# MayDomine/Burst-Attention

Hardware: NVIDIA H100
Metric: attention fwd+bwd TFLOPS/s (bs=1, H=32, d=128, bf16; seq in config, default 262144 on N > 1 GPUs, 65536 on one), aggregate over GPUs (higher is better)
Workload: dtype bf16

## Files before the change

burst-attention_b200/csrc/bwd_sm90.cu:

```cuda
#include <math.h>
#include <stdlib.h>

#include <mutex>
#include <vector>

#include "host_common.h"
#include "sm90_ptx.cuh"

namespace ba {

constexpr int kBwdThreads = 384;
constexpr int kBwdN = 128;
constexpr int kBwdM = 64;

struct BwdParams {
  const float* lse;
  int64_t lse_sb, lse_sh;
  const float* delta;
  int64_t dl_sb, dl_sh;
  float* dk_acc;
  int64_t dk_sb, dk_ss, dk_sh;
  float* dv_acc;
  int64_t dv_sb, dv_ss, dv_sh;
  int B, Sq, Sk, H;
  int G;
  float scale, scale_log2;
  int causal, causal_off;
  const float* bias;
  int64_t bias_sb, bias_sh;
  int* sem;
  int* ticket;
};

__device__ __forceinline__ int ld_acquire_gpu(const int* p) {
  int v;
  asm volatile("ld.acquire.gpu.global.s32 %0, [%1];" : "=r"(v) : "l"(p) : "memory");
  return v;
}
__device__ __forceinline__ void st_release_gpu(int* p, int v) {
  asm volatile("st.release.gpu.global.s32 [%0], %1;" ::"l"(p), "r"(v) : "memory");
}

struct __align__(8) BwdBarriers {
  uint64_t kv_full;
  uint64_t q_full[2], q_empty[2];
  int key_block;
};

template <int kD>
struct BwdLayout {
  static_assert(kD == 64 || kD == 128, "head dim 64 or 128");
  static constexpr int kBoxes = kD / 64;
  static constexpr int kBoxKV = kBwdN * 128;
  static constexpr int kBoxQ = kBwdM * 128;
  static constexpr int kOffK = 0;
  static constexpr int kOffV = kOffK + kBoxes * kBoxKV;
  static constexpr int kOffQ = kOffV + kBoxes * kBoxKV;
  static constexpr int kOffDO = kOffQ + 2 * kBoxes * kBoxQ;
  static constexpr int kOffDS = kOffDO + 2 * kBoxes * kBoxQ;
  static constexpr int kOffDQ = kOffDS + 2 * kBwdN * 128;
  static constexpr int kOffStat = kOffDQ + kBoxes * kBwdM * 64 * 4;
  static constexpr int kOffBar = kOffStat + 2 * 2 * kBwdM * 4;
  static constexpr int kSmemBytes = kOffBar + 64;
  static_assert(kSmemBytes <= 232448, "backward kernel exceeds 227 KiB of shared memory");
};

template <bool kBF16, int kD>
__global__ void __launch_bounds__(kBwdThreads, 1)
bwd_chunk_kernel(const __grid_constant__ CUtensorMap tmQ, const __grid_constant__ CUtensorMap tmK,
                 const __grid_constant__ CUtensorMap tmV, const __grid_constant__ CUtensorMap tmDO,
                 const __grid_constant__ CUtensorMap tmDQ, const BwdParams p) {
  extern __shared__ __align__(1024) uint8_t smem_raw[];
  uint8_t* smem = smem_raw;
  if ((smem_u32(smem) & 1023u) != 0) __trap();
  using L = BwdLayout<kD>;
  constexpr int kBoxes = L::kBoxes, kBoxKV = L::kBoxKV, kBoxQ = L::kBoxQ, kAcc = kD / 2;
  constexpr int kQStageB = kBoxes * kBoxQ;
  float* sStat = reinterpret_cast<float*>(smem + L::kOffStat);
  BwdBarriers* bars = reinterpret_cast<BwdBarriers*>(smem + L::kOffBar);

  const int warp = __shfl_sync(0xffffffffu, threadIdx.x >> 5, 0);
  const int lane = threadIdx.x & 31;
  const int hk = blockIdx.y, b = blockIdx.z;
  const int h0 = hk * p.G;
  int kb = blockIdx.x;
// ... 21 lines not shown
      mbar_init(&bars->q_empty[s], 8);
    }
    fence_mbar_init();
  }
  __syncthreads();

  if (warp < 4) {
    reg_alloc_dec<24>();
    if (warp != 0) return;
    if (lane == 0) {
      mbar_arrive_expect_tx(&bars->kv_full, 2 * kBoxes * kBoxKV);
      for (int half = 0; half < kBoxes; ++half) {
        tma_load_4d(smem + L::kOffK + half * kBoxKV, &tmK, &bars->kv_full, half * 64, hk, k0, b);
        tma_load_4d(smem + L::kOffV + half * kBoxKV, &tmV, &bars->kv_full, half * 64, hk, k0, b);
      }
    }
    int it = 0, h = h0;
    for (int step = 0; step < n_steps; ++step) {
      const int q0 = (i_begin + it) * kBwdM;
      const int st = step & 1;
      mbar_wait(&bars->q_empty[st], ((step >> 1) & 1) ^ 1);
      float* stat = sStat + st * 2 * kBwdM;
#pragma unroll
      for (int j = 0; j < 2; ++j) {
        const int row = q0 + lane + 32 * j;
        float l = INFINITY, dl = 0.f;
        if (row < p.Sq) {
          l = __ldg(p.lse + (int64_t)b * p.lse_sb + (int64_t)h * p.lse_sh + row);
          dl = __ldg(p.delta + (int64_t)b * p.dl_sb + (int64_t)h * p.dl_sh + row);
          if (l == -INFINITY) l = INFINITY;
        }
        stat[lane + 32 * j] = l * kLog2e;
        stat[kBwdM + lane + 32 * j] = dl;
      }
      __syncwarp();
      if (lane == 0) {
        mbar_arrive_expect_tx(&bars->q_full[st], 2 * kQStageB);
        for (int half = 0; half < kBoxes; ++half) {
          tma_load_4d(smem + L::kOffQ + st * kQStageB + half * kBoxQ, &tmQ, &bars->q_full[st], half * 64, h, q0, b);
          tma_load_4d(smem + L::kOffDO + st * kQStageB + half * kBoxQ, &tmDO, &bars->q_full[st], half * 64, h, q0, b);
        }
      }
      __syncwarp();
      if (++it == n_it) it = 0, ++h;
    }
    return;
  }

  reg_alloc_inc<240>();
  const int wg = (threadIdx.x >> 7) - 1;
  const int tid = threadIdx.x & 127;
  const int w = warp & 3, g = lane >> 2, t = lane & 3;
  const int kr_lo = wg * 64 + 16 * w + g;
  const int keys[2] = {k0 + kr_lo, k0 + kr_lo + 8};
  const float scale_log2 = p.scale_log2;
  float bias2[2];
  const bool reducer = kD == 128 || wg == 0;
  const int n_red = kD == 128 ? 2 : 1;

  float dk[kAcc], dv[kAcc];
#pragma unroll
  for (int i = 0; i < kAcc; ++i) dk[i] = dv[i] = 0.f;

  const uint32_t sK = smem_u32(smem + L::kOffK), sV = smem_u32(smem + L::kOffV);
  const uint32_t kw = wg * 64 * 128;
  float* sDQ = reinterpret_cast<float*>(smem + L::kOffDQ) + wg * kBwdM * 64;
  mbar_wait(&bars->kv_full, 0);
  int it = 0, h = h0;
  for (int step = 0; step < n_steps; ++step) {
    const int q0 = (i_begin + it) * kBwdM;
    const int st = step & 1;
    const uint32_t sQ = smem_u32(smem + L::kOffQ + st * kQStageB), sDO = smem_u32(smem + L::kOffDO + st * kQStageB);
    const float* stat = sStat + st * 2 * kBwdM;
    if (it == 0) {
#pragma unroll
      for (int r = 0; r < 2; ++r)
        bias2[r] = (p.bias && keys[r] < p.Sk)
                       ? __ldg(p.bias + (int64_t)b * p.bias_sb + (int64_t)h * p.bias_sh + keys[r]) * kLog2e
                       : 0.f;
    }
    mbar_wait(&bars->q_full[st], (step >> 1) & 1);

    float s[32], dp[32];
    wgmma_fence();
#pragma unroll
    for (int kk = 0; kk < kD / 16; ++kk) {
      const uint32_t okv = (kk >> 2) * kBoxKV + kw + (kk & 3) * 32, oq = (kk >> 2) * kBoxQ + (kk & 3) * 32;
      wgmma_ss_n64<kBF16, 0, 0>(s, make_desc(sK + okv, 16, 1024), make_desc(sQ + oq, 16, 1024), kk > 0 ? 1u : 0u);
    }
    wgmma_commit();
#pragma unroll
    for (int kk = 0; kk < kD / 16; ++kk) {
      const uint32_t okv = (kk >> 2) * kBoxKV + kw + (kk & 3) * 32, oq = (kk >> 2) * kBoxQ + (kk & 3) * 32;
      wgmma_ss_n64<kBF16, 0, 0>(dp, make_desc(sV + okv, 16, 1024), make_desc(sDO + oq, 16, 1024), kk > 0 ? 1u : 0u);
    }
    wgmma_commit();
    wgmma_wait<1>();
    fence_regs<32>(s);

    const bool need_mask = p.causal && (q0 + p.causal_off < k0 + kBwdN - 1);
    uint32_t pp[16], ds[16];
#pragma unroll
    for (int c = 0; c < 8; ++c) {
      const float2 l2 = *reinterpret_cast<const float2*>(stat + 8 * c + 2 * t);
#pragma unroll
      for (int r = 0; r < 2; ++r) {
        const int e = 4 * c + 2 * r;
        float p0 = ex2(fmaf(s[e], scale_log2, bias2[r] - l2.x));
        float p1 = ex2(fmaf(s[e + 1], scale_log2, bias2[r] - l2.y));
        if (keys[r] >= p.Sk) p0 = p1 = 0.f;
        if (need_mask) {
          const int q = q0 + 8 * c + 2 * t;
          if (q < keys[r] - p.causal_off) p0 = 0.f;
          if (q + 1 < keys[r] - p.causal_off) p1 = 0.f;
        }
        s[e] = p0, s[e + 1] = p1;
        pp[2 * c + r] = pack2<kBF16>(p0, p1);
      }
    }

    wgmma_wait<0>();
    fence_regs<32>(dp);
    fence_regs<16>(pp);
    fence_regs<kAcc>(dv);
    wgmma_fence();
#pragma unroll
    for (int kk = 0; kk < kBwdM / 16; ++kk) {
      const uint64_t d_do = make_desc(sDO + kk * 16 * 128, kBoxQ, 1024);
      if constexpr (kD == 128) wgmma_rs_n128<kBF16, 1>(dv, pp + 4 * kk, d_do, 1u);
      else wgmma_rs_n64<kBF16, 1>(dv, pp + 4 * kk, d_do, 1u);
    }
    wgmma_commit();

#pragma unroll
    for (int c = 0; c < 8; ++c) {
      const float2 dl = *reinterpret_cast<const float2*>(stat + kBwdM + 8 * c + 2 * t);
#pragma unroll
      for (int r = 0; r < 2; ++r) {
        const int e = 4 * c + 2 * r;
        ds[2 * c + r] = pack2<kBF16>(s[e] * (dp[e] - dl.x), s[e + 1] * (dp[e + 1] - dl.y));
      }
    }

    uint8_t* sDS = smem + L::kOffDS + st * kBwdN * 128;
#pragma unroll
    for (int c = 0; c < 8; ++c)
#pragma unroll
      for (int r = 0; r < 2; ++r) {
        const int kr = kr_lo + 8 * r;
        *reinterpret_cast<uint32_t*>(sDS + kr * 128 + ((c ^ (kr & 7)) << 4) + 4 * t) = ds[2 * c + r];
      }
    fence_proxy_async_smem();
    named_bar_sync(1, 256);

    float dq[32];
    fence_regs<16>(ds);
    fence_regs<kAcc>(dk);
    auto issue_dk = [&]() {
#pragma unroll
      for (int kk = 0; kk < kBwdM / 16; ++kk) {
        const uint64_t d_q = make_desc(sQ + kk * 16 * 128, kBoxQ, 1024);
        if constexpr (kD == 128) wgmma_rs_n128<kBF16, 1>(dk, ds + 4 * kk, d_q, 1u);
        else wgmma_rs_n64<kBF16, 1>(dk, ds + 4 * kk, d_q, 1u);
      }
      wgmma_commit();
    };
    if (reducer) {
      const uint32_t a0 = smem_u32(sDS), b0 = sK + wg * kBoxKV;
      wgmma_fence();
#pragma unroll
      for (int kk = 0; kk < kBwdN / 16; ++kk)
        wgmma_ss_n64<kBF16, 1, 1>(dq, make_desc(a0 + kk * 16 * 128, 8192, 1024),
                                  make_desc(b0 + kk * 16 * 128, kBoxKV, 1024), kk > 0 ? 1u : 0u);
      wgmma_commit();
      issue_dk();
      wgmma_wait<1>();
    } else {
      wgmma_fence();
      issue_dk();
      wgmma_wait<1>();
    }
    fence_regs<kAcc>(dv);
    fence_regs<16>(pp);

    if (reducer) {
      fence_regs<32>(dq);
      const uint32_t bar_id = 2 + wg;
      if (tid == 0) tma_store_wait_read<0>();
      named_bar_sync(bar_id, 128);
#pragma unroll
      for (int c = 0; c < 8; ++c)
#pragma unroll
        for (int r = 0; r < 2; ++r)
          *reinterpret_cast<float2*>(sDQ + (16 * w + g + 8 * r) * 64 + 8 * c + 2 * t) =
              make_float2(dq[4 * c + 2 * r] * p.scale, dq[4 * c + 2 * r + 1] * p.scale);
      fence_proxy_async_smem();
      named_bar_sync(bar_id, 128);
      if (tid == 0) {
        int* turn = p.sem ? p.sem + ((int64_t)b * p.H + h) * nQ + (i_begin + it) : nullptr;
        const int my_turn = kb * n_red + wg;
        if (turn) {
          while (ld_acquire_gpu(turn) != my_turn) __nanosleep(64);
        }
        tma_reduce_add_4d(&tmDQ, sDQ, wg * 64, h, q0, b);
        tma_store_commit();
        if (turn) {
          tma_store_wait<0>();
          __threadfence();
          st_release_gpu(turn, my_turn + 1);
        }
      }
    }
    wgmma_wait<0>();
    fence_regs<kAcc>(dk);
    fence_regs<16>(ds);
    __syncwarp();
    if (lane == 0) mbar_arrive(&bars->q_empty[st]);
    if (++it == n_it) it = 0, ++h;
  }
  if (reducer && tid == 0) tma_store_wait<0>();

#pragma unroll
  for (int r = 0; r < 2; ++r) {
    if (keys[r] >= p.Sk) continue;
    float* pk = p.dk_acc + (int64_t)b * p.dk_sb + (int64_t)keys[r] * p.dk_ss + (int64_t)hk * p.dk_sh + 2 * t;
    float* pv = p.dv_acc + (int64_t)b * p.dv_sb + (int64_t)keys[r] * p.dv_ss + (int64_t)hk * p.dv_sh + 2 * t;
#pragma unroll
    for (int c = 0; c < kD / 8; ++c) {
      float2 a = *reinterpret_cast<float2*>(pk + 8 * c);
      a.x = fmaf(dk[4 * c + 2 * r], p.scale, a.x);
      a.y = fmaf(dk[4 * c + 2 * r + 1], p.scale, a.y);
      *reinterpret_cast<float2*>(pk + 8 * c) = a;
      float2 v = *reinterpret_cast<float2*>(pv + 8 * c);
      v.x += dv[4 * c + 2 * r];
      v.y += dv[4 * c + 2 * r + 1];
      *reinterpret_cast<float2*>(pv + 8 * c) = v;
    }
  }
}

static int launch_bwd(int dtype, int D, const CUtensorMap& tmQ, const CUtensorMap& tmK, const CUtensorMap& tmV,
                      const CUtensorMap& tmDO, const CUtensorMap& tmDQ, const BwdParams& p, cudaStream_t stream) {
  const bool bf16 = dtype == BA_DTYPE_BF16;
  void (*kern)(CUtensorMap, CUtensorMap, CUtensorMap, CUtensorMap, CUtensorMap, BwdParams) =
      D == 64 ? (bf16 ? bwd_chunk_kernel<true, 64> : bwd_chunk_kernel<false, 64>)
              : (bf16 ? bwd_chunk_kernel<true, 128> : bwd_chunk_kernel<false, 128>);
  const int smem = D == 64 ? BwdLayout<64>::kSmemBytes : BwdLayout<128>::kSmemBytes;
  BA_CHECK_CUDA(cudaFuncSetAttribute(kern, cudaFuncAttributeMaxDynamicSharedMemorySize, smem));
  dim3 grid((p.Sk + kBwdN - 1) / kBwdN, p.H / p.G, p.B);
  kern<<<grid, kBwdThreads, smem, stream>>>(tmQ, tmK, tmV, tmDO, tmDQ, p);
  BA_CHECK_CUDA(cudaGetLastError());
  return BA_OK;
}

struct BwdWorkspace {
  int device;
  cudaStream_t stream;
  int* ptr;
  size_t cap;
};
static std::mutex g_ws_mutex;
static std::vector<BwdWorkspace> g_ws;

static int* bwd_sem_workspace(size_t n_ints, cudaStream_t stream) {
  int dev = 0;
  if (cudaGetDevice(&dev) != cudaSuccess) return nullptr;
  std::lock_guard<std::mutex> lock(g_ws_mutex);
  BwdWorkspace* w = nullptr;
  for (auto& e : g_ws)
    if (e.device == dev && e.stream == stream) w = &e;
  if (!w) {
    g_ws.push_back(BwdWorkspace{dev, stream, nullptr, 0});
    w = &g_ws.back();
  }
  if (w->cap < n_ints) {
    if (w->ptr && cudaFreeAsync(w->ptr, stream) != cudaSuccess) return nullptr;
    w->ptr = nullptr, w->cap = 0;
    if (cudaMallocAsync(reinterpret_cast<void**>(&w->ptr), n_ints * sizeof(int), stream) != cudaSuccess) return nullptr;
    w->cap = n_ints;
  }
  if (cudaMemsetAsync(w->ptr, 0, n_ints * sizeof(int), stream) != cudaSuccess) return nullptr;
  return w->ptr;
}

}

extern "C" int ba_bwd_chunk(ba_tensor4 d_o, ba_tensor4 q, ba_tensor4 k, ba_tensor4 v, ba_rowstat delta,
                            ba_rowstat lse, ba_tensor4 dq_acc, ba_tensor4 dk_acc, ba_tensor4 dv_acc, int B, int Sq,
                            int Sk, int H, int D, float scale, int mask_mode, int causal_offset, int flags, int dtype,
                            void* stream) {
  ba_rowstat none = {nullptr, 0, 0};
  return ba_bwd_chunk_bias(d_o, q, k, v, delta, lse, none, dq_acc, dk_acc, dv_acc, B, Sq, Sk, H, D, scale, mask_mode,
                           causal_offset, flags, dtype, stream);
}

extern "C" int ba_bwd_chunk_bias(ba_tensor4 d_o, ba_tensor4 q, ba_tensor4 k, ba_tensor4 v, ba_rowstat delta,
                                 ba_rowstat lse, ba_rowstat key_bias, ba_tensor4 dq_acc, ba_tensor4 dk_acc,
                                 ba_tensor4 dv_acc, int B, int Sq, int Sk, int H, int D, float scale, int mask_mode,
                                 int causal_offset, int flags, int dtype, void* stream) {
  return ba_bwd_chunk_gqa(d_o, q, k, v, delta, lse, key_bias, dq_acc, dk_acc, dv_acc, B, Sq, Sk, H, H, D, scale,
                          mask_mode, causal_offset, flags, dtype, stream);
}

extern "C" int ba_bwd_chunk_gqa(ba_tensor4 d_o, ba_tensor4 q, ba_tensor4 k, ba_tensor4 v, ba_rowstat delta,
                                ba_rowstat lse, ba_rowstat key_bias, ba_tensor4 dq_acc, ba_tensor4 dk_acc,
                                ba_tensor4 dv_acc, int B, int Sq, int Sk, int H, int H_kv, int D, float scale,
                                int mask_mode, int causal_offset, int flags, int dtype, void* stream) {
  using namespace ba;
  int rc;
  if ((rc = check_chunk_args("ba_bwd_chunk", B, Sq, Sk, H, H_kv, D, scale, mask_mode, dtype))) return rc;
  BA_REQUIRE(d_o.ptr && q.ptr && k.ptr && v.ptr && delta.ptr && lse.ptr, "ba_bwd_chunk: null input");
  BA_REQUIRE(dq_acc.ptr && dk_acc.ptr && dv_acc.ptr && aligned16(dq_acc, 4) && aligned16(dk_acc, 4) &&
                 aligned16(dv_acc, 4),
             "ba_bwd_chunk: fp32 accumulators must be non-null, 16-byte aligned, strides multiple of 4");

  CUtensorMap tmQ, tmK, tmV, tmDO, tmDQ;
  const CUtensorMapDataType dt = lowp_dtype(dtype);
  if ((rc = make_tensor_map(&tmQ, q, B, Sq, H, D, dt, 2, 64, kBwdM, true))) return rc;
  if ((rc = make_tensor_map(&tmDO, d_o, B, Sq, H, D, dt, 2, 64, kBwdM, true))) return rc;
  if ((rc = make_tensor_map(&tmK, k, B, Sk, H_kv, D, dt, 2, 64, kBwdN, true))) return rc;
  if ((rc = make_tensor_map(&tmV, v, B, Sk, H_kv, D, dt, 2, 64, kBwdN, true))) return rc;
  if ((rc = make_tensor_map(&tmDQ, dq_acc, B, Sq, H, D, CU_TENSOR_MAP_DATA_TYPE_FLOAT32, 4, 64, kBwdM, false)))
    return rc;

  BwdParams p;
  p.lse = lse.ptr, p.lse_sb = lse.stride_b, p.lse_sh = lse.stride_h;
  p.delta = delta.ptr, p.dl_sb = delta.stride_b, p.dl_sh = delta.stride_h;
  p.dk_acc = static_cast<float*>(dk_acc.ptr);
  p.dk_sb = dk_acc.stride_b, p.dk_ss = dk_acc.stride_s, p.dk_sh = dk_acc.stride_h;
  p.dv_acc = static_cast<float*>(dv_acc.ptr);
  p.dv_sb = dv_acc.stride_b, p.dv_ss = dv_acc.stride_s, p.dv_sh = dv_acc.stride_h;
  p.bias = key_bias.ptr, p.bias_sb = key_bias.stride_b, p.bias_sh = key_bias.stride_h;
  p.B = B, p.Sq = Sq, p.Sk = Sk, p.H = H;
  p.G = H / H_kv;
  p.scale = scale;
  p.scale_log2 = scale * kLog2e;
  p.causal = mask_mode == BA_MASK_CAUSAL;
  p.causal_off = causal_offset;
  cudaStream_t st = static_cast<cudaStream_t>(stream);
  p.sem = p.ticket = nullptr;
  if (flags & BA_BWD_DETERMINISTIC) {
    const size_t n_turn = (size_t)B * H * ((Sq + kBwdM - 1) / kBwdM);
    const size_t n = n_turn + (size_t)B * H_kv;
    p.sem = bwd_sem_workspace(n, st);
    if (p.sem) p.ticket = p.sem + n_turn;
    if (!p.sem) {
      set_error("ba_bwd_chunk: could not allocate the deterministic-mode workspace (%zu ints)", n);
      return BA_ERR_CUDA;
    }
  }
  return launch_bwd(dtype, D, tmQ, tmK, tmV, tmDO, tmDQ, p, st);
}
```

burst-attention_b200/csrc/sm90_ptx.cuh:

```cuda
#pragma once
#include <cuda.h>
#include <cuda_bf16.h>
#include <cuda_fp16.h>
#include <cuda_runtime.h>
#include <stdint.h>

namespace ba {

#define BA_DEVICE __device__ __forceinline__

BA_DEVICE uint32_t smem_u32(const void* p) {
  return static_cast<uint32_t>(__cvta_generic_to_shared(p));
}
constexpr float kLog2e = 1.4426950408889634f;
constexpr float kLn2 = 0.6931471805599453f;
BA_DEVICE float ex2(float x) {
  float y;
  asm("ex2.approx.ftz.f32 %0, %1;" : "=f"(y) : "f"(x));
  return y;
}
BA_DEVICE float lg2(float x) {
  float y;
  asm("lg2.approx.ftz.f32 %0, %1;" : "=f"(y) : "f"(x));
  return y;
// ... 61 lines not shown
  asm volatile("prefetch.tensormap [%0];" ::"l"(reinterpret_cast<uint64_t>(m)) : "memory");
}
BA_DEVICE void tma_load_4d(void* smem_dst, const CUtensorMap* m, uint64_t* bar, int c0, int c1, int c2,
                           int c3) {
  asm volatile(
      "cp.async.bulk.tensor.4d.shared::cluster.global.mbarrier::complete_tx::bytes"
      " [%0], [%1, {%3, %4, %5, %6}], [%2];"
      :
      : "r"(smem_u32(smem_dst)), "l"(reinterpret_cast<uint64_t>(m)), "r"(smem_u32(bar)), "r"(c0), "r"(c1),
        "r"(c2), "r"(c3)
      : "memory");
}
BA_DEVICE void tma_reduce_add_4d(const CUtensorMap* m, const void* smem_src, int c0, int c1, int c2, int c3) {
  asm volatile(
      "cp.reduce.async.bulk.tensor.4d.global.shared::cta.add.tile.bulk_group [%0, {%2, %3, %4, %5}], [%1];"
      :
      : "l"(reinterpret_cast<uint64_t>(m)), "r"(smem_u32(smem_src)), "r"(c0), "r"(c1), "r"(c2), "r"(c3)
      : "memory");
}
BA_DEVICE void tma_store_commit() { asm volatile("cp.async.bulk.commit_group;" ::: "memory"); }
template <int N>
BA_DEVICE void tma_store_wait_read() {
  asm volatile("cp.async.bulk.wait_group.read %0;" ::"n"(N) : "memory");
}
template <int N>
BA_DEVICE void tma_store_wait() {
  asm volatile("cp.async.bulk.wait_group %0;" ::"n"(N) : "memory");
}

BA_DEVICE uint64_t make_desc(uint32_t smem_addr, uint32_t lbo_bytes, uint32_t sbo_bytes) {
  uint64_t d = 0;
  d |= static_cast<uint64_t>((smem_addr & 0x3FFFF) >> 4);
  d |= static_cast<uint64_t>((lbo_bytes >> 4) & 0x3FFF) << 16;
  d |= static_cast<uint64_t>((sbo_bytes >> 4) & 0x3FFF) << 32;
  d |= static_cast<uint64_t>(1) << 62;
  return d;
}

BA_DEVICE void wgmma_fence() { asm volatile("wgmma.fence.sync.aligned;" ::: "memory"); }
BA_DEVICE void wgmma_commit() { asm volatile("wgmma.commit_group.sync.aligned;" ::: "memory"); }
template <int N>
BA_DEVICE void wgmma_wait() {
  asm volatile("wgmma.wait_group.sync.aligned %0;" ::"n"(N) : "memory");
}
template <int N>
BA_DEVICE void fence_regs(float* r) {
#pragma unroll
  for (int i = 0; i < N; ++i) asm volatile("" : "+f"(r[i])::"memory");
}
template <int N>
BA_DEVICE void fence_regs(uint32_t* r) {
#pragma unroll
  for (int i = 0; i < N; ++i) asm volatile("" : "+r"(r[i])::"memory");
}

#define BA_WGMMA_ACC_64(d) "+f"(d[0]), "+f"(d[1]), "+f"(d[2]), "+f"(d[3]), "+f"(d[4]), "+f"(d[5]), "+f"(d[6]), "+f"(d[7]), "+f"(d[8]), "+f"(d[9]), "+f"(d[10]), "+f"(d[11]), "+f"(d[12]), "+f"(d[13]), "+f"(d[14]), "+f"(d[15]), "+f"(d[16]), "+f"(d[17]), "+f"(d[18]), "+f"(d[19]), "+f"(d[20]), "+f"(d[21]), "+f"(d[22]), "+f"(d[23]), "+f"(d[24]), "+f"(d[25]), "+f"(d[26]), "+f"(d[27]), "+f"(d[28]), "+f"(d[29]), "+f"(d[30]), "+f"(d[31])
#define BA_WGMMA_ACC_128(d) BA_WGMMA_ACC_64(d), "+f"(d[32]), "+f"(d[33]), "+f"(d[34]), "+f"(d[35]), "+f"(d[36]), "+f"(d[37]), "+f"(d[38]), "+f"(d[39]), "+f"(d[40]), "+f"(d[41]), "+f"(d[42]), "+f"(d[43]), "+f"(d[44]), "+f"(d[45]), "+f"(d[46]), "+f"(d[47]), "+f"(d[48]), "+f"(d[49]), "+f"(d[50]), "+f"(d[51]), "+f"(d[52]), "+f"(d[53]), "+f"(d[54]), "+f"(d[55]), "+f"(d[56]), "+f"(d[57]), "+f"(d[58]), "+f"(d[59]), "+f"(d[60]), "+f"(d[61]), "+f"(d[62]), "+f"(d[63])
#define BA_WGMMA_REGS_64 "%0,%1,%2,%3,%4,%5,%6,%7,%8,%9,%10,%11,%12,%13,%14,%15,%16,%17,%18,%19,%20,%21,%22,%23,%24,%25,%26,%27,%28,%29,%30,%31"
#define BA_WGMMA_REGS_128 BA_WGMMA_REGS_64 ",%32,%33,%34,%35,%36,%37,%38,%39,%40,%41,%42,%43,%44,%45,%46,%47,%48,%49,%50,%51,%52,%53,%54,%55,%56,%57,%58,%59,%60,%61,%62,%63"
#define BA_WGMMA_SS(N, TY, A, B, SC, TA, TB)                                                     \
  asm volatile("{\n\t.reg .pred p;\n\t"                                                        \
               "setp.ne.b32 p, %" #SC ", 0;\n\t"                                               \
               "wgmma.mma_async.sync.aligned.m64n" #N "k16.f32." TY "." TY " "                 \
               "{" BA_WGMMA_REGS_##N "}, "                                                      \
               "%" #A ", %" #B ", p, 1, 1, %" #TA ", %" #TB ";\n\t}\n"                         \
               : BA_WGMMA_ACC_##N(d)                                                            \
               : "l"(a_desc), "l"(b_desc), "r"(scale_d), "n"(kTA), "n"(kTB))
#define BA_WGMMA_RS(N, TY, A0, A1, A2, A3, B, SC, TB)                                            \
  asm volatile("{\n\t.reg .pred p;\n\t"                                                        \
               "setp.ne.b32 p, %" #SC ", 0;\n\t"                                               \
               "wgmma.mma_async.sync.aligned.m64n" #N "k16.f32." TY "." TY " "                 \
               "{" BA_WGMMA_REGS_##N "}, "                                                      \
               "{%" #A0 ",%" #A1 ",%" #A2 ",%" #A3 "}, %" #B ", p, 1, 1, %" #TB ";\n\t}\n"     \
               : BA_WGMMA_ACC_##N(d)                                                            \
               : "r"(a[0]), "r"(a[1]), "r"(a[2]), "r"(a[3]), "l"(b_desc), "r"(scale_d), "n"(kTB))

template <bool kBF16, int kTA, int kTB>
BA_DEVICE void wgmma_ss_n64(float* d, uint64_t a_desc, uint64_t b_desc, uint32_t scale_d) {
  if constexpr (kBF16) BA_WGMMA_SS(64, "bf16", 32, 33, 34, 35, 36);
  else BA_WGMMA_SS(64, "f16", 32, 33, 34, 35, 36);
}
template <bool kBF16, int kTB>
BA_DEVICE void wgmma_rs_n64(float* d, const uint32_t* a, uint64_t b_desc, uint32_t scale_d) {
  if constexpr (kBF16) BA_WGMMA_RS(64, "bf16", 32, 33, 34, 35, 36, 37, 38);
  else BA_WGMMA_RS(64, "f16", 32, 33, 34, 35, 36, 37, 38);
}
template <bool kBF16, int kTA, int kTB>
BA_DEVICE void wgmma_ss_n128(float* d, uint64_t a_desc, uint64_t b_desc, uint32_t scale_d) {
  if constexpr (kBF16) BA_WGMMA_SS(128, "bf16", 64, 65, 66, 67, 68);
  else BA_WGMMA_SS(128, "f16", 64, 65, 66, 67, 68);
}
template <bool kBF16, int kTB>
BA_DEVICE void wgmma_rs_n128(float* d, const uint32_t* a, uint64_t b_desc, uint32_t scale_d) {
  if constexpr (kBF16) BA_WGMMA_RS(128, "bf16", 64, 65, 66, 67, 68, 69, 70);
  else BA_WGMMA_RS(128, "f16", 64, 65, 66, 67, 68, 69, 70);
}

template <bool kBF16>
BA_DEVICE uint32_t pack2(float lo, float hi) {
  if constexpr (kBF16) {
    __nv_bfloat162 v = __floats2bfloat162_rn(lo, hi);
    return *reinterpret_cast<uint32_t*>(&v);
  } else {
    __half2 v = __floats2half2_rn(lo, hi);
    return *reinterpret_cast<uint32_t*>(&v);
  }
// ... 4 lines not shown
```

burst-attention_b200/csrc/fwd_sm90.cu:

```cuda
#include <math.h>
#include <stdlib.h>

#include "host_common.h"
#include "sm90_ptx.cuh"

namespace ba {

constexpr int kBlockM = 128;
constexpr int kBlockN = 128;
constexpr int kKStages = 2;
constexpr int kVStages = 2;
constexpr int kBoxBytes = 128 * 64 * 2;
constexpr int kFwdThreads = 384;

struct FwdParams {
  float* o_acc;
  int64_t oacc_sb, oacc_ss, oacc_sh;
  float* lse;
  int64_t lse_sb, lse_sh;
  void* o_out;
  int64_t oout_sb, oout_ss, oout_sh;
  int B, Sq, Sk, H;
  int G;
  float scale_log2;
// ... 101 lines not shown
        }
        __syncwarp();
        if (lane == 0) mbar_arrive(&bars->b_full[ks]);
      }
      if (lane == 0) {
        const int vs = i % kVStages, vph = (i / kVStages) & 1;
        mbar_wait(&bars->v_empty[vs], vph ^ 1);
        mbar_arrive_expect_tx(&bars->v_full[vs], kTileBytes);
        for (int half = 0; half < kBoxes; ++half)
          tma_load_4d(sV + vs * kTileBytes + half * kBoxBytes, &tmV, &bars->v_full[vs], half * 64, hk,
                      i * kBlockN, b);
      }
      __syncwarp();
    }
    return;
  }

  reg_alloc_inc<232>();
  const int wg = (threadIdx.x >> 7) - 1;
  const int w = warp & 3, g = lane >> 2, t = lane & 3;
  const int r_lo = row0 + wg * 64 + 16 * w + g;
  const int rows[2] = {r_lo, r_lo + 8};
  const int n_mine = fwd_trip_count(row0 + wg * 64, p);
  const float scale_log2 = p.scale_log2;
  int limit[2];
#pragma unroll
  for (int r = 0; r < 2; ++r) limit[r] = p.causal ? min(rows[r] + p.causal_off, p.Sk - 1) : p.Sk - 1;
  const int limit_min = min(limit[0], limit[1]);

  float o[kOReg];
  float m[2] = {-INFINITY, -INFINITY}, l[2] = {0.f, 0.f};
#pragma unroll
  for (int i = 0; i < kOReg; ++i) o[i] = 0.f;
  if (p.load_state) {
#pragma unroll
    for (int r = 0; r < 2; ++r) {
      if (rows[r] >= p.Sq) continue;
      const float lse_prev = p.lse[(int64_t)b * p.lse_sb + (int64_t)h * p.lse_sh + rows[r]];
      if (lse_prev != -INFINITY) {
        m[r] = lse_prev * kLog2e;
        l[r] = t == 0 ? 1.f : 0.f;
      }
      const float* src = p.o_acc + (int64_t)b * p.oacc_sb + (int64_t)rows[r] * p.oacc_ss + (int64_t)h * p.oacc_sh;
#pragma unroll
      for (int c = 0; c < kD / 8; ++c) {
        const float2 f = __ldg(reinterpret_cast<const float2*>(src + 8 * c + 2 * t));
        o[4 * c + 2 * r] = f.x;
        o[4 * c + 2 * r + 1] = f.y;
      }
    }
  }

  const uint32_t q_base = smem_u32(sQ) + wg * 64 * 128;
  mbar_wait(&bars->q_full, 0);
  for (int i = 0; i < n_tiles; ++i) {
    const int ks = i % kKStages, kph = (i / kKStages) & 1;
    const int vs = i % kVStages, vph = (i / kVStages) & 1;
    const bool work = i < n_mine;
    mbar_wait(&bars->k_full[ks], kph);
    float sc[64];
    if (work) {
      const uint32_t k_base = smem_u32(sK + ks * kTileBytes);
      wgmma_fence();
#pragma unroll
      for (int kk = 0; kk < kD / 16; ++kk) {
        const uint32_t off = (kk >> 2) * kBoxBytes + (kk & 3) * 32;
        wgmma_ss_n128<kBF16, 0, 0>(sc, make_desc(q_base + off, 16, 1024), make_desc(k_base + off, 16, 1024),
                                   kk > 0 ? 1u : 0u);
      }
      wgmma_commit();
      wgmma_wait<0>();
      fence_regs<64>(sc);
      const int key0 = i * kBlockN;
      if constexpr (kBias) {
        mbar_wait(&bars->b_full[ks], kph);
        const float* bias = sBias + ks * kBlockN;
#pragma unroll
        for (int c = 0; c < 16; ++c) {
          const float2 bb = *reinterpret_cast<const float2*>(bias + 8 * c + 2 * t);
#pragma unroll
          for (int r = 0; r < 2; ++r) {
            sc[4 * c + 2 * r] = fmaf(sc[4 * c + 2 * r], scale_log2, bb.x);
            sc[4 * c + 2 * r + 1] = fmaf(sc[4 * c + 2 * r + 1], scale_log2, bb.y);
          }
        }
      } else {
#pragma unroll
        for (int j = 0; j < 64; ++j) sc[j] *= scale_log2;
      }
      if (key0 + kBlockN - 1 > limit_min) {
#pragma unroll
        for (int c = 0; c < 16; ++c)
#pragma unroll
          for (int e = 0; e < 4; ++e)
            if (key0 + 8 * c + 2 * t + (e & 1) > limit[e >> 1]) sc[4 * c + e] = -INFINITY;
      }
    }
    __syncwarp();
    if (lane == 0) mbar_arrive(&bars->k_empty[ks]);
    if (work) {
      uint32_t pa[32];
#pragma unroll
      for (int r = 0; r < 2; ++r) {
        float mx = -INFINITY;
#pragma unroll
        for (int c = 0; c < 16; ++c) mx = fmaxf(mx, fmaxf(sc[4 * c + 2 * r], sc[4 * c + 2 * r + 1]));
        mx = fmaxf(mx, __shfl_xor_sync(0xffffffffu, mx, 1));
        mx = fmaxf(mx, __shfl_xor_sync(0xffffffffu, mx, 2));
        const float m_new = fmaxf(m[r], mx);
        const float f = (m[r] == -INFINITY) ? 0.f : ex2(m[r] - m_new);
        const float neg_m = (m_new == -INFINITY) ? 0.f : -m_new;
        m[r] = m_new;
        float sum = 0.f;
#pragma unroll
        for (int c = 0; c < 16; ++c) {
          const float p0 = ex2(sc[4 * c + 2 * r] + neg_m), p1 = ex2(sc[4 * c + 2 * r + 1] + neg_m);
          sc[4 * c + 2 * r] = p0;
          sc[4 * c + 2 * r + 1] = p1;
          sum += p0 + p1;
        }
        l[r] = l[r] * f + sum;
#pragma unroll
        for (int c = 0; c < kD / 8; ++c) {
          o[4 * c + 2 * r] *= f;
          o[4 * c + 2 * r + 1] *= f;
        }
      }
#pragma unroll
      for (int j = 0; j < 32; ++j) pa[j] = pack2<kBF16>(sc[2 * j], sc[2 * j + 1]);
      mbar_wait(&bars->v_full[vs], vph);
      const uint32_t v_base = smem_u32(sV + vs * kTileBytes);
      fence_regs<32>(pa);
      fence_regs<kOReg>(o);
      wgmma_fence();
#pragma unroll
      for (int kk = 0; kk < kBlockN / 16; ++kk) {
        const uint64_t dv = make_desc(v_base + kk * 16 * 128, kBoxBytes, 1024);
        if constexpr (kD == 128) wgmma_rs_n128<kBF16, 1>(o, pa + 4 * kk, dv, 1u);
        else wgmma_rs_n64<kBF16, 1>(o, pa + 4 * kk, dv, 1u);
      }
      wgmma_commit();
      wgmma_wait<0>();
      fence_regs<kOReg>(o);
    } else {
      mbar_wait(&bars->v_full[vs], vph);
    }
    __syncwarp();
    if (lane == 0) mbar_arrive(&bars->v_empty[vs]);
  }

#pragma unroll
  for (int r = 0; r < 2; ++r) {
    float lr = l[r];
    lr += __shfl_xor_sync(0xffffffffu, lr, 1);
    lr += __shfl_xor_sync(0xffffffffu, lr, 2);
    const int row = rows[r];
    if (row >= p.Sq) continue;
    const float inv_l = lr > 0.f ? 1.f / lr : 0.f;
    if (t == 0) p.lse[(int64_t)b * p.lse_sb + (int64_t)h * p.lse_sh + row] = lr > 0.f ? (m[r] + lg2(lr)) * kLn2 : -INFINITY;
    if (p.store_lowp) {
      uint16_t* dst = reinterpret_cast<uint16_t*>(p.o_out) + (int64_t)b * p.oout_sb + (int64_t)row * p.oout_ss +
                      (int64_t)h * p.oout_sh + 2 * t;
#pragma unroll
      for (int c = 0; c < kD / 8; ++c)
        *reinterpret_cast<uint32_t*>(dst + 8 * c) = pack2<kBF16>(o[4 * c + 2 * r] * inv_l, o[4 * c + 2 * r + 1] * inv_l);
    } else {
      float* dst = p.o_acc + (int64_t)b * p.oacc_sb + (int64_t)row * p.oacc_ss + (int64_t)h * p.oacc_sh + 2 * t;
#pragma unroll
      for (int c = 0; c < kD / 8; ++c)
        *reinterpret_cast<float2*>(dst + 8 * c) = make_float2(o[4 * c + 2 * r] * inv_l, o[4 * c + 2 * r + 1] * inv_l);
    }
  }
}


static int launch_fwd(int dtype, int D, bool bias, const CUtensorMap& tmQ, const CUtensorMap& tmK,
                      const CUtensorMap& tmV, const FwdParams& p, cudaStream_t stream) {
  const bool bf16 = dtype == BA_DTYPE_BF16;
  void (*kern)(CUtensorMap, CUtensorMap, CUtensorMap, FwdParams);
  if (bias)
    kern = D == 64 ? (bf16 ? fwd_chunk_kernel<true, 64, true> : fwd_chunk_kernel<false, 64, true>)
                   : (bf16 ? fwd_chunk_kernel<true, 128, true> : fwd_chunk_kernel<false, 128, true>);
  else
    kern = D == 64 ? (bf16 ? fwd_chunk_kernel<true, 64, false> : fwd_chunk_kernel<false, 64, false>)
                   : (bf16 ? fwd_chunk_kernel<true, 128, false> : fwd_chunk_kernel<false, 128, false>);
  const int smem = D == 64 ? FwdLayout<64>::kSmemBytes : FwdLayout<128>::kSmemBytes;
  BA_CHECK_CUDA(cudaFuncSetAttribute(kern, cudaFuncAttributeMaxDynamicSharedMemorySize, smem));
  dim3 grid((p.Sq + kBlockM - 1) / kBlockM, p.H, p.B);
  kern<<<grid, kFwdThreads, smem, stream>>>(tmQ, tmK, tmV, p);
  BA_CHECK_CUDA(cudaGetLastError());
  return BA_OK;
}

}

extern "C" int ba_fwd_chunk(ba_tensor4 q, ba_tensor4 k, ba_tensor4 v, ba_tensor4 o_acc, ba_rowstat lse,
                            ba_tensor4 o_out, int B, int Sq, int Sk, int H, int D, float scale, int mask_mode,
                            int causal_offset, int flags, int dtype, void* stream) {
  ba_rowstat none = {nullptr, 0, 0};
  return ba_fwd_chunk_bias(q, k, v, none, o_acc, lse, o_out, B, Sq, Sk, H, D, scale, mask_mode, causal_offset, flags,
                           dtype, stream);
// ... 48 lines not shown
```

Measured before the change: 472.5.

## Prefetch next step's S/dP WGMMAs before dK wait and swizzle dQ staging

Restructures the backward consumer loop so the S and dP WGMMAs for the next Q tile are issued before waiting on the current dK GEMM, overlapping tensor-core work across steps. It also changes the dQ shared-memory staging to a 128B-swizzled layout with two 32-column TMA reduce-adds, aimed at cutting bank conflicts on the float2 stores. Forget_regs hints let the compiler drop the s/dp registers early, and an optional compile-time phase-clock instrumentation path is added. The extra in-flight accumulators raise register pressure and could cause spills.

After: 484.2, median of 6. +2.5%, better.

```diff
diff --git a/burst-attention_b200/csrc/bwd_sm90.cu b/burst-attention_b200/csrc/bwd_sm90.cu
--- a/burst-attention_b200/csrc/bwd_sm90.cu
+++ b/burst-attention_b200/csrc/bwd_sm90.cu
@@ -30,7 +30,23 @@
   int64_t bias_sb, bias_sh;
   int* sem;
   int* ticket;
+#ifdef BA_BWD_PHASES
+  unsigned* phase_clk;
+#endif
 };
+
+#ifdef BA_BWD_PHASES
+enum BwdPhase { kPhStart, kPhQFull, kPhS, kPhP, kPhDP, kPhDS, kPhBar, kPhDQ, kPhStaged, kPhDK, kBwdPhasePts };
+__device__ __forceinline__ unsigned clock_now() {
+  unsigned t;
+  asm volatile("mov.u32 %0, %%clock;" : "=r"(t)::"memory");
+  return t;
+}
+static unsigned* g_phase_clk = nullptr;
+constexpr bool kDkFromSmem = true;
+#else
+constexpr bool kDkFromSmem = false;
+#endif
 
 __device__ __forceinline__ int ld_acquire_gpu(const int* p) {
   int v;
@@ -158,7 +174,7 @@
   const int tid = threadIdx.x & 127;
   const int w = warp & 3, g = lane >> 2, t = lane & 3;
   const int kr_lo = wg * 64 + 16 * w + g;
-  const int keys[2] = {k0 + kr_lo, k0 + kr_lo + 8};
+  const int key0 = k0 + kr_lo;
   const float scale_log2 = p.scale_log2;
   float bias2[2];
   const bool reducer = kD == 128 || wg == 0;
@@ -171,38 +187,52 @@
   const uint32_t sK = smem_u32(smem + L::kOffK), sV = smem_u32(smem + L::kOffV);
   const uint32_t kw = wg * 64 * 128;
   float* sDQ = reinterpret_cast<float*>(smem + L::kOffDQ) + wg * kBwdM * 64;
+#ifdef BA_BWD_PHASES
+  const int clk0 = (p.phase_clk && hk == 0 && b == 0 && tid == 0)
+                       ? ((int)blockIdx.x * 2 + wg) * n_steps * kBwdPhasePts
+                       : -1;
+#define BA_PHASE(step, pt) \
+  if (clk0 >= 0) p.phase_clk[clk0 + (step) * kBwdPhasePts + (pt)] = clock_now()
+#else
+#define BA_PHASE(step, pt)
+#endif
   mbar_wait(&bars->kv_full, 0);
+  float s[32], dp[32];
+  auto issue_s_dp = [&](int st) {
+    const uint32_t sQ = smem_u32(smem + L::kOffQ + st * kQStageB), sDO = smem_u32(smem + L::kOffDO + st * kQStageB);
+    wgmma_fence();
+#pragma unroll
+    for (int kk = 0; kk < kD / 16; ++kk) {
+      const uint32_t okv = (kk >> 2) * kBoxKV + kw + (kk & 3) * 32, oq = (kk >> 2) * kBoxQ + (kk & 3) * 32;
+      wgmma_ss_n64<kBF16, 0, 0>(s, make_desc(sK + okv, 16, 1024), make_desc(sQ + oq, 16, 1024), kk > 0 ? 1u : 0u);
+    }
+    wgmma_commit();
+#pragma unroll
+    for (int kk = 0; kk < kD / 16; ++kk) {
+      const uint32_t okv = (kk >> 2) * kBoxKV + kw + (kk & 3) * 32, oq = (kk >> 2) * kBoxQ + (kk & 3) * 32;
+      wgmma_ss_n64<kBF16, 0, 0>(dp, make_desc(sV + okv, 16, 1024), make_desc(sDO + oq, 16, 1024), kk > 0 ? 1u : 0u);
+    }
+    wgmma_commit();
+  };
+  mbar_wait(&bars->q_full[0], 0);
+  issue_s_dp(0);
   int it = 0, h = h0;
-  for (int step = 0; step < n_steps; ++step) {
+  for (int step = 0;; ++step) {
     const int q0 = (i_begin + it) * kBwdM;
     const int st = step & 1;
     const uint32_t sQ = smem_u32(smem + L::kOffQ + st * kQStageB), sDO = smem_u32(smem + L::kOffDO + st * kQStageB);
     const float* stat = sStat + st * 2 * kBwdM;
+    BA_PHASE(step, kPhStart);
     if (it == 0) {
 #pragma unroll
       for (int r = 0; r < 2; ++r)
-        bias2[r] = (p.bias && keys[r] < p.Sk)
-                       ? __ldg(p.bias + (int64_t)b * p.bias_sb + (int64_t)h * p.bias_sh + keys[r]) * kLog2e
+        bias2[r] = (p.bias && (key0 + 8 * r) < p.Sk)
+                       ? __ldg(p.bias + (int64_t)b * p.bias_sb + (int64_t)h * p.bias_sh + (key0 + 8 * r)) * kLog2e
                        : 0.f;
     }
-    mbar_wait(&bars->q_full[st], (step >> 1) & 1);
-
-    float s[32], dp[32];
-    wgmma_fence();
-#pragma unroll
-    for (int kk = 0; kk < kD / 16; ++kk) {
-      const uint32_t okv = (kk >> 2) * kBoxKV + kw + (kk & 3) * 32, oq = (kk >> 2) * kBoxQ + (kk & 3) * 32;
-      wgmma_ss_n64<kBF16, 0, 0>(s, make_desc(sK + okv, 16, 1024), make_desc(sQ + oq, 16, 1024), kk > 0 ? 1u : 0u);
-    }
-    wgmma_commit();
-#pragma unroll
-    for (int kk = 0; kk < kD / 16; ++kk) {
-      const uint32_t okv = (kk >> 2) * kBoxKV + kw + (kk & 3) * 32, oq = (kk >> 2) * kBoxQ + (kk & 3) * 32;
-      wgmma_ss_n64<kBF16, 0, 0>(dp, make_desc(sV + okv, 16, 1024), make_desc(sDO + oq, 16, 1024), kk > 0 ? 1u : 0u);
-    }
-    wgmma_commit();
     wgmma_wait<1>();
     fence_regs<32>(s);
+    BA_PHASE(step, kPhS);
 
     const bool need_mask = p.causal && (q0 + p.causal_off < k0 + kBwdN - 1);
     uint32_t pp[16], ds[16];
@@ -214,19 +244,21 @@
         const int e = 4 * c + 2 * r;
         float p0 = ex2(fmaf(s[e], scale_log2, bias2[r] - l2.x));
         float p1 = ex2(fmaf(s[e + 1], scale_log2, bias2[r] - l2.y));
-        if (keys[r] >= p.Sk) p0 = p1 = 0.f;
+        if ((key0 + 8 * r) >= p.Sk) p0 = p1 = 0.f;
         if (need_mask) {
           const int q = q0 + 8 * c + 2 * t;
-          if (q < keys[r] - p.causal_off) p0 = 0.f;
-          if (q + 1 < keys[r] - p.causal_off) p1 = 0.f;
+          if (q < (key0 + 8 * r) - p.causal_off) p0 = 0.f;
+          if (q + 1 < (key0 + 8 * r) - p.causal_off) p1 = 0.f;
         }
         s[e] = p0, s[e + 1] = p1;
         pp[2 * c + r] = pack2<kBF16>(p0, p1);
       }
     }
+    BA_PHASE(step, kPhP);
 
     wgmma_wait<0>();
     fence_regs<32>(dp);
+    BA_PHASE(step, kPhDP);
     fence_regs<16>(pp);
     fence_regs<kAcc>(dv);
     wgmma_fence();
@@ -247,6 +279,8 @@
         ds[2 * c + r] = pack2<kBF16>(s[e] * (dp[e] - dl.x), s[e + 1] * (dp[e + 1] - dl.y));
       }
     }
+    forget_regs<32>(s);
+    forget_regs<32>(dp);
 
     uint8_t* sDS = smem + L::kOffDS + st * kBwdN * 128;
 #pragma unroll
@@ -257,7 +291,9 @@
         *reinterpret_cast<uint32_t*>(sDS + kr * 128 + ((c ^ (kr & 7)) << 4) + 4 * t) = ds[2 * c + r];
       }
     fence_proxy_async_smem();
+    BA_PHASE(step, kPhDS);
     named_bar_sync(1, 256);
+    BA_PHASE(step, kPhBar);
 
     float dq[32];
     fence_regs<16>(ds);
@@ -266,8 +302,14 @@
 #pragma unroll
       for (int kk = 0; kk < kBwdM / 16; ++kk) {
         const uint64_t d_q = make_desc(sQ + kk * 16 * 128, kBoxQ, 1024);
-        if constexpr (kD == 128) wgmma_rs_n128<kBF16, 1>(dk, ds + 4 * kk, d_q, 1u);
-        else wgmma_rs_n64<kBF16, 1>(dk, ds + 4 * kk, d_q, 1u);
+        if constexpr (kDkFromSmem) {
+          const uint64_t d_ds = make_desc(smem_u32(sDS) + kw + kk * 32, 16, 1024);
+          if constexpr (kD == 128) wgmma_ss_n128<kBF16, 0, 1>(dk, d_ds, d_q, 1u);
+          else wgmma_ss_n64<kBF16, 0, 1>(dk, d_ds, d_q, 1u);
+        } else {
+          if constexpr (kD == 128) wgmma_rs_n128<kBF16, 1>(dk, ds + 4 * kk, d_q, 1u);
+          else wgmma_rs_n64<kBF16, 1>(dk, ds + 4 * kk, d_q, 1u);
+        }
       }
       wgmma_commit();
     };
@@ -288,27 +330,35 @@
     }
     fence_regs<kAcc>(dv);
     fence_regs<16>(pp);
+    BA_PHASE(step, kPhDQ);
 
     if (reducer) {
       fence_regs<32>(dq);
       const uint32_t bar_id = 2 + wg;
       if (tid == 0) tma_store_wait_read<0>();
       named_bar_sync(bar_id, 128);
-#pragma unroll
-      for (int c = 0; c < 8; ++c)
-#pragma unroll
-        for (int r = 0; r < 2; ++r)
-          *reinterpret_cast<float2*>(sDQ + (16 * w + g + 8 * r) * 64 + 8 * c + 2 * t) =
-              make_float2(dq[4 * c + 2 * r] * p.scale, dq[4 * c + 2 * r + 1] * p.scale);
+      const bool odd = g & 1;
+      uint8_t* const row = reinterpret_cast<uint8_t*>(sDQ) + (16 * w + g) * 128 + 8 * (t & 1);
+      const int x = ((t >> 1) ^ g ^ (odd ? 4 : 0)) << 4;
+#pragma unroll
+      for (int k = 0; k < 8; ++k)
+#pragma unroll
+        for (int r = 0; r < 2; ++r) {
+          const int e0 = 4 * k + 2 * r, e1 = 4 * (k ^ 2) + 2 * r;
+          const float v0 = odd ? dq[e1] : dq[e0], v1 = odd ? dq[e1 + 1] : dq[e0 + 1];
+          *reinterpret_cast<float2*>(row + (k >> 2) * (kBwdM * 128) + r * 8 * 128 + ((32 * (k & 3)) ^ x)) =
+              make_float2(v0 * p.scale, v1 * p.scale);
+        }
       fence_proxy_async_smem();
       named_bar_sync(bar_id, 128);
       if (tid == 0) {
         int* turn = p.sem ? p.sem + ((int64_t)b * p.H + h) * nQ + (i_begin + it) : nullptr;
-        const int my_turn = kb * n_red + wg;
+        const int my_turn = turn ? bars->key_block * n_red + wg : 0;
         if (turn) {
           while (ld_acquire_gpu(turn) != my_turn) __nanosleep(64);
         }
         tma_reduce_add_4d(&tmDQ, sDQ, wg * 64, h, q0, b);
+        tma_reduce_add_4d(&tmDQ, sDQ + kBwdM * 32, wg * 64 + 32, h, q0, b);
         tma_store_commit();
         if (turn) {
           tma_store_wait<0>();
@@ -316,21 +366,31 @@
           st_release_gpu(turn, my_turn + 1);
         }
       }
-    }
-    wgmma_wait<0>();
+      BA_PHASE(step, kPhStaged);
+    }
+
+    if (it + 1 == n_it && h + 1 == h0 + p.G) break;
+    mbar_wait(&bars->q_full[st ^ 1], ((step + 1) >> 1) & 1);
+    BA_PHASE(step, kPhQFull);
+    issue_s_dp(st ^ 1);
+    wgmma_wait<2>();
     fence_regs<kAcc>(dk);
-    fence_regs<16>(ds);
+    if constexpr (!kDkFromSmem) fence_regs<16>(ds);
+    BA_PHASE(step, kPhDK);
     __syncwarp();
     if (lane == 0) mbar_arrive(&bars->q_empty[st]);
     if (++it == n_it) it = 0, ++h;
   }
+  wgmma_wait<0>();
+  fence_regs<kAcc>(dk);
+  BA_PHASE(n_steps - 1, kPhDK);
   if (reducer && tid == 0) tma_store_wait<0>();
 
 #pragma unroll
   for (int r = 0; r < 2; ++r) {
-    if (keys[r] >= p.Sk) continue;
-    float* pk = p.dk_acc + (int64_t)b * p.dk_sb + (int64_t)keys[r] * p.dk_ss + (int64_t)hk * p.dk_sh + 2 * t;
-    float* pv = p.dv_acc + (int64_t)b * p.dv_sb + (int64_t)keys[r] * p.dv_ss + (int64_t)hk * p.dv_sh + 2 * t;
+    if ((key0 + 8 * r) >= p.Sk) continue;
+    float* pk = p.dk_acc + (int64_t)b * p.dk_sb + (int64_t)(key0 + 8 * r) * p.dk_ss + (int64_t)hk * p.dk_sh + 2 * t;
+    float* pv = p.dv_acc + (int64_t)b * p.dv_sb + (int64_t)(key0 + 8 * r) * p.dv_ss + (int64_t)hk * p.dv_sh + 2 * t;
 #pragma unroll
     for (int c = 0; c < kD / 8; ++c) {
       float2 a = *reinterpret_cast<float2*>(pk + 8 * c);
@@ -391,6 +451,10 @@
 
 }
 
+#ifdef BA_BWD_PHASES
+extern "C" void ba_bwd_set_phase_buffer(unsigned* clk) { ba::g_phase_clk = clk; }
+#endif
+
 extern "C" int ba_bwd_chunk(ba_tensor4 d_o, ba_tensor4 q, ba_tensor4 k, ba_tensor4 v, ba_rowstat delta,
                             ba_rowstat lse, ba_tensor4 dq_acc, ba_tensor4 dk_acc, ba_tensor4 dv_acc, int B, int Sq,
                             int Sk, int H, int D, float scale, int mask_mode, int causal_offset, int flags, int dtype,
@@ -426,7 +490,7 @@
   if ((rc = make_tensor_map(&tmDO, d_o, B, Sq, H, D, dt, 2, 64, kBwdM, true))) return rc;
   if ((rc = make_tensor_map(&tmK, k, B, Sk, H_kv, D, dt, 2, 64, kBwdN, true))) return rc;
   if ((rc = make_tensor_map(&tmV, v, B, Sk, H_kv, D, dt, 2, 64, kBwdN, true))) return rc;
-  if ((rc = make_tensor_map(&tmDQ, dq_acc, B, Sq, H, D, CU_TENSOR_MAP_DATA_TYPE_FLOAT32, 4, 64, kBwdM, false)))
+  if ((rc = make_tensor_map(&tmDQ, dq_acc, B, Sq, H, D, CU_TENSOR_MAP_DATA_TYPE_FLOAT32, 4, 32, kBwdM, true)))
     return rc;
 
   BwdParams p;
@@ -445,6 +509,9 @@
   p.causal_off = causal_offset;
   cudaStream_t st = static_cast<cudaStream_t>(stream);
   p.sem = p.ticket = nullptr;
+#ifdef BA_BWD_PHASES
+  p.phase_clk = g_phase_clk;
+#endif
   if (flags & BA_BWD_DETERMINISTIC) {
     const size_t n_turn = (size_t)B * H * ((Sq + kBwdM - 1) / kBwdM);
     const size_t n = n_turn + (size_t)B * H_kv;
diff --git a/burst-attention_b200/csrc/sm90_ptx.cuh b/burst-attention_b200/csrc/sm90_ptx.cuh
--- a/burst-attention_b200/csrc/sm90_ptx.cuh
+++ b/burst-attention_b200/csrc/sm90_ptx.cuh
@@ -137,6 +137,11 @@
 BA_DEVICE void fence_regs(uint32_t* r) {
 #pragma unroll
   for (int i = 0; i < N; ++i) asm volatile("" : "+r"(r[i])::"memory");
+}
+template <int N>
+BA_DEVICE void forget_regs(float* r) {
+#pragma unroll
+  for (int i = 0; i < N; ++i) asm volatile("" : "=f"(r[i]));
 }
 
 #define BA_WGMMA_ACC_64(d) "+f"(d[0]), "+f"(d[1]), "+f"(d[2]), "+f"(d[3]), "+f"(d[4]), "+f"(d[5]), "+f"(d[6]), "+f"(d[7]), "+f"(d[8]), "+f"(d[9]), "+f"(d[10]), "+f"(d[11]), "+f"(d[12]), "+f"(d[13]), "+f"(d[14]), "+f"(d[15]), "+f"(d[16]), "+f"(d[17]), "+f"(d[18]), "+f"(d[19]), "+f"(d[20]), "+f"(d[21]), "+f"(d[22]), "+f"(d[23]), "+f"(d[24]), "+f"(d[25]), "+f"(d[26]), "+f"(d[27]), "+f"(d[28]), "+f"(d[29]), "+f"(d[30]), "+f"(d[31])
```

## Overlap softmax with next QK^T and previous PV wgmma in forward consumer loop

Applied to the files above, without the earlier changes.

Restructures the consumer warpgroup loop into a software pipeline: the S=QK^T wgmma for tile i and the PV wgmma for tile i-1 are issued together, and softmax for tile i runs while the PV GEMM is in flight. The aim is to hide softmax ALU/exp latency behind tensor core work, as in FlashAttention-3 intra-warpgroup pipelining. It also skips the O rescale when every row's correction factor is 1 across the warp. The change keeps more registers live (sc, pa and o at the same time), which risks spills. Non-working tiles are now drained in a separate loop.

Result: faster. 470.0 before, 479.1 after (median of 6 runs) (+1.9%).

```diff
diff --git a/burst-attention_b200/csrc/fwd_sm90.cu b/burst-attention_b200/csrc/fwd_sm90.cu
--- a/burst-attention_b200/csrc/fwd_sm90.cu
+++ b/burst-attention_b200/csrc/fwd_sm90.cu
@@ -177,101 +177,141 @@
   }
 
   const uint32_t q_base = smem_u32(sQ) + wg * 64 * 128;
+  float sc[64];
+  uint32_t pa[32];
+  float f[2];
+  auto wait_k = [&](int i) {
+    mbar_wait(&bars->k_full[i % kKStages], (i / kKStages) & 1);
+    if constexpr (kBias) mbar_wait(&bars->b_full[i % kKStages], (i / kKStages) & 1);
+  };
+  auto wait_v = [&](int i) { mbar_wait(&bars->v_full[i % kVStages], (i / kVStages) & 1); };
+  auto arrive = [&](uint64_t* bar) {
+    __syncwarp();
+    if (lane == 0) mbar_arrive(bar);
+  };
+  auto issue_s = [&](int i) {
+    const uint32_t k_base = smem_u32(sK + (i % kKStages) * kTileBytes);
+#pragma unroll
+    for (int kk = 0; kk < kD / 16; ++kk) {
+      const uint32_t off = (kk >> 2) * kBoxBytes + (kk & 3) * 32;
+      wgmma_ss_n128<kBF16, 0, 0>(sc, make_desc(q_base + off, 16, 1024), make_desc(k_base + off, 16, 1024),
+                                 kk > 0 ? 1u : 0u);
+    }
+    wgmma_commit();
+  };
+  auto issue_pv = [&](int i) {
+    const uint32_t v_base = smem_u32(sV + (i % kVStages) * kTileBytes);
+#pragma unroll
+    for (int kk = 0; kk < kBlockN / 16; ++kk) {
+      const uint64_t dv = make_desc(v_base + kk * 16 * 128, kBoxBytes, 1024);
+      if constexpr (kD == 128) wgmma_rs_n128<kBF16, 1>(o, pa + 4 * kk, dv, 1u);
+      else wgmma_rs_n64<kBF16, 1>(o, pa + 4 * kk, dv, 1u);
+    }
+    wgmma_commit();
+  };
+  auto softmax = [&](int i) {
+    const int ks = i % kKStages, key0 = i * kBlockN;
+    if constexpr (kBias) {
+      const float* bias = sBias + ks * kBlockN;
+#pragma unroll
+      for (int c = 0; c < 16; ++c) {
+        const float2 bb = *reinterpret_cast<const float2*>(bias + 8 * c + 2 * t);
+#pragma unroll
+        for (int r = 0; r < 2; ++r) {
+          sc[4 * c + 2 * r] = fmaf(sc[4 * c + 2 * r], scale_log2, bb.x);
+          sc[4 * c + 2 * r + 1] = fmaf(sc[4 * c + 2 * r + 1], scale_log2, bb.y);
+        }
+      }
+    } else {
+#pragma unroll
+      for (int j = 0; j < 64; ++j) sc[j] *= scale_log2;
+    }
+    if (key0 + kBlockN - 1 > limit_min) {
+#pragma unroll
+      for (int c = 0; c < 16; ++c)
+#pragma unroll
+        for (int e = 0; e < 4; ++e)
+          if (key0 + 8 * c + 2 * t + (e & 1) > limit[e >> 1]) sc[4 * c + e] = -INFINITY;
+    }
+#pragma unroll
+    for (int r = 0; r < 2; ++r) {
+      float mx = -INFINITY;
+#pragma unroll
+      for (int c = 0; c < 16; ++c) mx = fmaxf(mx, fmaxf(sc[4 * c + 2 * r], sc[4 * c + 2 * r + 1]));
+      mx = fmaxf(mx, __shfl_xor_sync(0xffffffffu, mx, 1));
+      mx = fmaxf(mx, __shfl_xor_sync(0xffffffffu, mx, 2));
+      const float m_new = fmaxf(m[r], mx);
+      f[r] = (m[r] == -INFINITY) ? 0.f : ex2(m[r] - m_new);
+      const float neg_m = (m_new == -INFINITY) ? 0.f : -m_new;
+      m[r] = m_new;
+      float sum = 0.f;
+#pragma unroll
+      for (int c = 0; c < 16; ++c) {
+        const float p0 = ex2(sc[4 * c + 2 * r] + neg_m), p1 = ex2(sc[4 * c + 2 * r + 1] + neg_m);
+        sc[4 * c + 2 * r] = p0;
+        sc[4 * c + 2 * r + 1] = p1;
+        sum += p0 + p1;
+      }
+      l[r] = l[r] * f[r] + sum;
+    }
+    __syncwarp();
+    if (lane == 0 && !(fminf(l[0], l[1]) < 0.f)) mbar_arrive(&bars->k_empty[ks]);
+  };
+  auto rescale_and_pack = [&]() {
+    if (!__all_sync(0xffffffffu, f[0] == 1.f && f[1] == 1.f)) {
+#pragma unroll
+      for (int r = 0; r < 2; ++r)
+#pragma unroll
+        for (int c = 0; c < kD / 8; ++c) {
+          o[4 * c + 2 * r] *= f[r];
+          o[4 * c + 2 * r + 1] *= f[r];
+        }
+    }
+#pragma unroll
+    for (int j = 0; j < 32; ++j) pa[j] = pack2<kBF16>(sc[2 * j], sc[2 * j + 1]);
+  };
+
   mbar_wait(&bars->q_full, 0);
-  for (int i = 0; i < n_tiles; ++i) {
-    const int ks = i % kKStages, kph = (i / kKStages) & 1;
-    const int vs = i % kVStages, vph = (i / kVStages) & 1;
-    const bool work = i < n_mine;
-    mbar_wait(&bars->k_full[ks], kph);
-    float sc[64];
-    if (work) {
-      const uint32_t k_base = smem_u32(sK + ks * kTileBytes);
-      wgmma_fence();
-#pragma unroll
-      for (int kk = 0; kk < kD / 16; ++kk) {
-        const uint32_t off = (kk >> 2) * kBoxBytes + (kk & 3) * 32;
-        wgmma_ss_n128<kBF16, 0, 0>(sc, make_desc(q_base + off, 16, 1024), make_desc(k_base + off, 16, 1024),
-                                   kk > 0 ? 1u : 0u);
-      }
-      wgmma_commit();
-      wgmma_wait<0>();
+  if (n_mine > 0) {
+    wait_k(0);
+    wgmma_fence();
+    issue_s(0);
+    wgmma_wait<0>();
+    fence_regs<64>(sc);
+    softmax(0);
+    rescale_and_pack();
+    for (int i = 1; i < n_mine; ++i) {
+      wait_k(i);
+      wait_v(i - 1);
       fence_regs<64>(sc);
-      const int key0 = i * kBlockN;
-      if constexpr (kBias) {
-        mbar_wait(&bars->b_full[ks], kph);
-        const float* bias = sBias + ks * kBlockN;
-#pragma unroll
-        for (int c = 0; c < 16; ++c) {
-          const float2 bb = *reinterpret_cast<const float2*>(bias + 8 * c + 2 * t);
-#pragma unroll
-          for (int r = 0; r < 2; ++r) {
-            sc[4 * c + 2 * r] = fmaf(sc[4 * c + 2 * r], scale_log2, bb.x);
-            sc[4 * c + 2 * r + 1] = fmaf(sc[4 * c + 2 * r + 1], scale_log2, bb.y);
-          }
-        }
-      } else {
-#pragma unroll
-        for (int j = 0; j < 64; ++j) sc[j] *= scale_log2;
-      }
-      if (key0 + kBlockN - 1 > limit_min) {
-#pragma unroll
-        for (int c = 0; c < 16; ++c)
-#pragma unroll
-          for (int e = 0; e < 4; ++e)
-            if (key0 + 8 * c + 2 * t + (e & 1) > limit[e >> 1]) sc[4 * c + e] = -INFINITY;
-      }
-    }
-    __syncwarp();
-    if (lane == 0) mbar_arrive(&bars->k_empty[ks]);
-    if (work) {
-      uint32_t pa[32];
-#pragma unroll
-      for (int r = 0; r < 2; ++r) {
-        float mx = -INFINITY;
-#pragma unroll
-        for (int c = 0; c < 16; ++c) mx = fmaxf(mx, fmaxf(sc[4 * c + 2 * r], sc[4 * c + 2 * r + 1]));
-        mx = fmaxf(mx, __shfl_xor_sync(0xffffffffu, mx, 1));
-        mx = fmaxf(mx, __shfl_xor_sync(0xffffffffu, mx, 2));
-        const float m_new = fmaxf(m[r], mx);
-        const float f = (m[r] == -INFINITY) ? 0.f : ex2(m[r] - m_new);
-        const float neg_m = (m_new == -INFINITY) ? 0.f : -m_new;
-        m[r] = m_new;
-        float sum = 0.f;
-#pragma unroll
-        for (int c = 0; c < 16; ++c) {
-          const float p0 = ex2(sc[4 * c + 2 * r] + neg_m), p1 = ex2(sc[4 * c + 2 * r + 1] + neg_m);
-          sc[4 * c + 2 * r] = p0;
-          sc[4 * c + 2 * r + 1] = p1;
-          sum += p0 + p1;
-        }
-        l[r] = l[r] * f + sum;
-#pragma unroll
-        for (int c = 0; c < kD / 8; ++c) {
-          o[4 * c + 2 * r] *= f;
-          o[4 * c + 2 * r + 1] *= f;
-        }
-      }
-#pragma unroll
-      for (int j = 0; j < 32; ++j) pa[j] = pack2<kBF16>(sc[2 * j], sc[2 * j + 1]);
-      mbar_wait(&bars->v_full[vs], vph);
-      const uint32_t v_base = smem_u32(sV + vs * kTileBytes);
       fence_regs<32>(pa);
       fence_regs<kOReg>(o);
       wgmma_fence();
-#pragma unroll
-      for (int kk = 0; kk < kBlockN / 16; ++kk) {
-        const uint64_t dv = make_desc(v_base + kk * 16 * 128, kBoxBytes, 1024);
-        if constexpr (kD == 128) wgmma_rs_n128<kBF16, 1>(o, pa + 4 * kk, dv, 1u);
-        else wgmma_rs_n64<kBF16, 1>(o, pa + 4 * kk, dv, 1u);
-      }
-      wgmma_commit();
+      issue_s(i);
+      issue_pv(i - 1);
+      wgmma_wait<1>();
+      fence_regs<64>(sc);
+      softmax(i);
       wgmma_wait<0>();
       fence_regs<kOReg>(o);
-    } else {
-      mbar_wait(&bars->v_full[vs], vph);
-    }
-    __syncwarp();
-    if (lane == 0) mbar_arrive(&bars->v_empty[vs]);
+      fence_regs<32>(pa);
+      arrive(&bars->v_empty[(i - 1) % kVStages]);
+      rescale_and_pack();
+    }
+    wait_v(n_mine - 1);
+    fence_regs<32>(pa);
+    fence_regs<kOReg>(o);
+    wgmma_fence();
+    issue_pv(n_mine - 1);
+    wgmma_wait<0>();
+    fence_regs<kOReg>(o);
+    arrive(&bars->v_empty[(n_mine - 1) % kVStages]);
+  }
+  for (int i = n_mine; i < n_tiles; ++i) {
+    mbar_wait(&bars->k_full[i % kKStages], (i / kKStages) & 1);
+    arrive(&bars->k_empty[i % kKStages]);
+    wait_v(i);
+    arrive(&bars->v_empty[i % kVStages]);
   }
 
 #pragma unroll
```
